# LPD-EPFL/ByzantineMomentum

Hardware: AMD Instinct MI355X
Metric: aggregations/sec (Byzantine-robust GAR over n workers x d dims; achieved HBM GB/s per GAR in roofline/per_gar) (higher is better)
Workload: dtype f32

## Files before the change

### byzantinemomentum_amd/csrc/anticge.hip

```cpp
#include "rank_body.h"
#include "table_sum.h"

namespace bm {

constexpr int kAcgScaleBlock = 256;
constexpr int kAcgMaxBlocks = 256 * 32;
constexpr Caps kAcgCaps = caps_of(kAcgMaxBlocks);
constexpr int kAcgScaleBlocks = 2048;

__global__ __launch_bounds__(64) void anticge_rank_kernel(const double* __restrict__ row_sq, int h, int maxpos,
                                                          int32_t* __restrict__ order, int32_t* __restrict__ order_out,
                                                          double* __restrict__ scal_out) {
  __shared__ double keys[BM_MAX_ROWS];
  __shared__ int32_t ranked[BM_MAX_ROWS];
  const int i = threadIdx.x;
  double key = i < h ? row_sq[i] : 0.0;
  if (!(__builtin_fabs(key) < __builtin_inf())) key = __builtin_inf();
  stable_argsort_body(key, h, keys, ranked);
  __syncthreads();
  order[i] = i < h ? ranked[i] : 0;
  if (order_out != nullptr) order_out[i] = i < h ? ranked[i] : 0;
  if (i == 0) scal_out[1] = keys[ranked[maxpos]];
}

template <int VEC>
__global__ __launch_bounds__(kTableBlock) void anticge_sum_kernel(RowTable rows, const int32_t* __restrict__ order,
                                                                int maxpos, int64_t nvec, float* __restrict__ out,
                                                                int tail, double* __restrict__ partial) {
  __shared__ const float* sel[BM_MAX_ROWS];
  __shared__ double red[kTableBlock / 64];
  const int m = maxpos > 0 ? maxpos : 1;
  if ((int)threadIdx.x < m) sel[threadIdx.x] = rows.p[load_index_coherent(order + threadIdx.x) & (BM_MAX_ROWS - 1)];
  __syncthreads();
  double wide = 0.0;
  table_sum_plain<VEC>(sel, m, nvec, tail, out, AnticgeFold{maxpos > 0}, [&](float x) { wide += (double)x * (double)x; });
  const double r = block_reduce_sum<kTableBlock>(wide, red);
  if (threadIdx.x == 0) partial[blockIdx.x] = r;
}

__global__ __launch_bounds__(64) void anticge_finish_kernel(const double* __restrict__ partial, int nparts,
                                                            double* __restrict__ scal_out) {
  const int lane = threadIdx.x;
  double tot = 0.0;
  for (int b = lane; b < nparts; b += 64) tot += partial[b];
#pragma unroll
  for (int off = 32; off > 0; off >>= 1) tot += __shfl_down(tot, off, 64);
  if (lane == 0) scal_out[0] = tot;
}

__device__ __forceinline__ bool anticge_multiplier(const double* __restrict__ scal, float* mult) {
  const float attnorm = (float)sqrt(scal[0]);
  if (!(attnorm > 0.0f)) return false;
  const float byznorm = (float)sqrt(scal[1]);
  const double norm = (__builtin_fabsf(byznorm) < __builtin_inff()) ? (double)byznorm : __builtin_inf();
  *mult = (float)(-nextafter(norm, 0.0) / (double)attnorm);
  return true;
}

template <int VEC>
__global__ __launch_bounds__(kAcgScaleBlock) void anticge_scale_kernel(float* __restrict__ vec, int64_t nvec,
                                                                  const double* __restrict__ scal) {
  float mult;
  if (!anticge_multiplier(scal, &mult)) return;
  using T = typename VecLoad<VEC>::T;
  const int64_t stride = (int64_t)gridDim.x * kAcgScaleBlock;
  for (int64_t v = (int64_t)blockIdx.x * kAcgScaleBlock + threadIdx.x; v < nvec; v += stride) {
    T x = *reinterpret_cast<const T*>(vec + v * VEC);
    if constexpr (VEC == 1) {
      x = x * mult;
    } else {
#pragma unroll
      for (int c = 0; c < VEC; ++c) x[c] = x[c] * mult;
    }
    *reinterpret_cast<T*>(vec + v * VEC) = x;
  }
}

constexpr int64_t kAcgOrderBytes = BM_MAX_ROWS * (int64_t)sizeof(int32_t);

}

extern "C" int64_t bm_anticge_workspace_bytes(int64_t d) {
  using namespace bm;
  if (d < 0) return BM_EINVAL;
  const int64_t pieces = piece_count(d) > 0 ? piece_count(d) : 1;
  return kAcgOrderBytes + pieces * kAcgCaps.sets() * (int64_t)sizeof(double);
}

extern "C" int bm_anticge_sum(const float* const* rows, int h, int64_t d, int f_decl, const double* row_sq,
                              float* sum_out, int32_t* order_out, double* scal_out, void* ws, void* stream) {
  using namespace bm;
  if (rows == nullptr || row_sq == nullptr || scal_out == nullptr || ws == nullptr || h < 1 || h > BM_MAX_ROWS ||
      f_decl < 1 || f_decl > h || d < 0 || (d > 0 && sum_out == nullptr))
    return BM_EINVAL;
  for (int i = 0; i < h && d > 0; ++i)
    if (rows[i] == nullptr) return BM_EINVAL;
  hipStream_t s = static_cast<hipStream_t>(stream);
  const int maxpos = h - f_decl;
  int32_t* order = static_cast<int32_t*>(ws);
  double* partial = reinterpret_cast<double*>(static_cast<char*>(ws) + kAcgOrderBytes);
  hipLaunchKernelGGL(anticge_rank_kernel, dim3(1), dim3(64), 0, s, row_sq, h, maxpos, order, order_out, scal_out);
  BM_LAUNCH_CHECK();
  RowTable tab{};
  for (int i = 0; i < h; ++i) tab.p[i] = rows[i];
  const int vec = Alignment().of(rows, h).of(sum_out).vec();
  int nparts = 0;
  const int rc = for_pieces(d, [&](int64_t lo, int64_t dp) {
    return for_body_and_tail<4>(Tail::kRidesNarrowed, vec, dp, kTableBlock, kAcgCaps, [&](auto width, const Span& sp) {
      hipLaunchKernelGGL(anticge_sum_kernel<decltype(width)::value>, dim3(sp.grid), dim3(kTableBlock), 0, s,
                         tab.advanced(lo), order, maxpos, sp.count, sum_out + lo, sp.tail, partial + sp.part);
      BM_LAUNCH_CHECK();
      return 0;
    }, &nparts);
  });
  if (rc != 0) return rc;
  hipLaunchKernelGGL(anticge_finish_kernel, dim3(1), dim3(64), 0, s, partial, nparts, scal_out);
  BM_LAUNCH_CHECK();
  return 0;
}

extern "C" int bm_anticge_scale(float* vec, int64_t d, const double* scal, void* stream) {
  using namespace bm;
  if (scal == nullptr || d < 0 || (d > 0 && vec == nullptr)) return BM_EINVAL;
  if (d == 0) return 0;
  hipStream_t s = static_cast<hipStream_t>(stream);
  return for_body_and_tail<4>(Tail::kOwnLaunch, Alignment().of(vec).vec(), d, kAcgScaleBlock, caps_of(kAcgScaleBlocks),
                              [&](auto width, const Span& sp) {
    hipLaunchKernelGGL(anticge_scale_kernel<decltype(width)::value>, dim3(sp.grid), dim3(kAcgScaleBlock), 0, s,
                       vec + sp.first, sp.count, scal);
    BM_LAUNCH_CHECK();
    return 0;
  });
}
```

### byzantinemomentum_amd/csrc/api.cpp

```cpp
#include <stdlib.h>
#include <string.h>
#include <math.h>
#include <algorithm>
#include <vector>
#include "bm_common.h"

namespace bm {
static int env_int(const char* name, int dflt) {
  const char* v = getenv(name);
  if (v == nullptr || *v == '\0') return dflt;
  return atoi(v);
}
static double env_double(const char* name, double dflt) {
  const char* v = getenv(name);
  if (v == nullptr || *v == '\0') return dflt;
  return atof(v);
}
Tuning& tuning_mutable() {
  static Tuning t = {env_int("BM_COL_BURST", 8),  env_int("BM_MEAN_BURST", 8),
                           env_int("BM_STEP_BURST", 8), env_int("BM_STEP_STREAM", 0), env_int("BM_PAIR_MODE", 0),
                           env_int("BM_PAIR_PLANES", 0), env_int("BM_PAIR_DITHER", 0), env_double("BM_PAIR_TAU", 2e-3),
                           env_int("BM_STUDY_BURST", 8), env_int("BM_STEP_STAGGER_US", 0),
                           env_int("BM_GRAM_STEADY", 1), env_int("BM_BULYAN_SHORT", 1),
                           env_int("BM_PAIR_LOAD_NT", 1), env_int("BM_RANK_ALGO", 0), env_int("BM_COL_WIDE", 1), env_int("BM_BRUTE_BUDGET", 0),
                           env_int("BM_WSUM_PIECE", 0), env_int("BM_SPECTRAL_LANES", 0),
                           env_int("BM_PERTURB_GRID", 0)};
  return t;
}
const Tuning& tuning() { return tuning_mutable(); }
}

extern "C" int bm_abi_version(void) { return 23; }

extern "C" int bm_tuning_set(const char* name, int value) {
  using namespace bm;
  if (name == nullptr) return BM_EINVAL;
  Tuning& t = tuning_mutable();
  const struct { const char* key; int* slot; } knobs[] = {
      {"BM_COL_BURST", &t.col_burst}, {"BM_MEAN_BURST", &t.mean_burst}, {"BM_STEP_BURST", &t.step_burst},
      {"BM_STEP_STREAM", &t.step_stream}, {"BM_PAIR_MODE", &t.pair_mode}, {"BM_PAIR_PLANES", &t.pair_planes},
      {"BM_PAIR_DITHER", &t.pair_dither}, {"BM_STUDY_BURST", &t.study_burst},
      {"BM_STEP_STAGGER_US", &t.step_stagger_us}, {"BM_GRAM_STEADY", &t.gram_steady},
      {"BM_BULYAN_SHORT", &t.bulyan_short}, {"BM_PAIR_LOAD_NT", &t.pair_load_nt},
      {"BM_RANK_ALGO", &t.rank_algo}, {"BM_COL_WIDE", &t.col_wide}, {"BM_BRUTE_BUDGET", &t.brute_budget},
      {"BM_WSUM_PIECE", &t.wsum_piece}, {"BM_SPECTRAL_LANES", &t.spectral_lanes},
      {"BM_PERTURB_GRID", &t.perturb_grid}};
  for (const auto& k : knobs)
    if (strcmp(name, k.key) == 0) {
      *k.slot = value;
      return 0;
    }
  return BM_EINVAL;
}

extern "C" const char* bm_error_string(int code) {
  if (code == 0) return "success";
  if (code == BM_EINVAL) return "invalid argument for libbm_gar";
  if (code == BM_ENOCOMM) return "RCCL is not available in this process (librccl.so.1 could not be bound)";
  if (code == BM_ECOMM) return "an RCCL call failed";
  if (code < 0) return hipGetErrorString(static_cast<hipError_t>(-code));
  return "unknown libbm_gar status";
}

namespace {
struct BruteGraph {
  int n;
  uint64_t adj[BM_MAX_ROWS];

  void build(const double* dist, double t) {
    for (int i = 0; i < n; ++i) adj[i] = 0;
    for (int i = 0; i < n; ++i)
      for (int j = i + 1; j < n; ++j) {
        const double v = dist[i * n + j];
        if (isfinite(v) && v <= t) {
          adj[i] |= (uint64_t)1 << j;
          adj[j] |= (uint64_t)1 << i;
        }
      }
  }

  bool has_clique(uint64_t cand, int need) const {
    const int count = __builtin_popcountll(cand);
    if (count < need) return false;
    if (need <= 1) return true;
    int worst = -1, worst_missing = 0;
    for (uint64_t rest = cand; rest != 0; rest &= rest - 1) {
      const int u = __builtin_ctzll(rest);
      const int missing = __builtin_popcountll(cand & ~adj[u] & ~((uint64_t)1 << u));
      if (missing > worst_missing) {
        worst = u;
        worst_missing = missing;
      }
    }
    if (worst < 0) return true;
    const int budget = count - need;
    if (budget == 0) return false;
    const uint64_t bit = (uint64_t)1 << worst;
    if (worst_missing <= budget && has_clique(cand & (adj[worst] | bit), need)) return true;
    return has_clique(cand & ~bit, need);
  }
};
}

extern "C" int bm_brute_select(const double* dist_nxn, int n, int f, int32_t* sel_out) {
  if (dist_nxn == nullptr || sel_out == nullptr || n < 1 || n > BM_MAX_ROWS || f < 0 || n - f < 1)
    return BM_EINVAL;
  const int k = n - f;
  const uint64_t everyone = n == 64 ? ~(uint64_t)0 : (((uint64_t)1 << n) - 1);
  std::vector<double> values;
  values.reserve((size_t)n * (n - 1) / 2 + 1);
  values.push_back(0.0);
  for (int i = 0; i < n; ++i)
    for (int j = i + 1; j < n; ++j) {
      const double v = dist_nxn[i * n + j];
      if (isfinite(v) && v > 0.0) values.push_back(v);
    }
  std::sort(values.begin(), values.end());
  values.erase(std::unique(values.begin(), values.end()), values.end());
  BruteGraph g;
  g.n = n;
  g.build(dist_nxn, values.back());
  if (!g.has_clique(everyone, k)) return BM_EINVAL;
  size_t lo = 0, hi = values.size() - 1;
  while (lo < hi) {
    const size_t mid = (lo + hi) / 2;
    g.build(dist_nxn, values[mid]);
    if (g.has_clique(everyone, k))
      hi = mid;
    else
      lo = mid + 1;
  }
  g.build(dist_nxn, values[lo]);
  uint64_t cand = everyone;
  int chosen = 0;
  for (int c = 0; c < n && chosen < k; ++c) {
    const uint64_t bit = (uint64_t)1 << c;
    if ((cand & bit) == 0) continue;
    const uint64_t above = c == 63 ? 0 : ~(((uint64_t)1 << (c + 1)) - 1);
    const uint64_t next = cand & g.adj[c] & above;
    if (g.has_clique(next, k - chosen - 1)) {
      sel_out[chosen++] = c;
      cand = next;
    }
  }
  return chosen == k ? 0 : BM_EINVAL;
}
```

### byzantinemomentum_amd/csrc/bm_common.h

```cpp
#pragma once
#include <hip/hip_runtime.h>
#include <stdint.h>
#include <utility>
#include "../../include/bm_gar.h"
#include "launch_plan.h"

namespace bm {

struct RowTable {
  const float* p[BM_MAX_ROWS];
  RowTable advanced(int64_t by) const {
    RowTable t = *this;
    advance(t.p, by);
    return t;
  }
};

static inline int hip_code(hipError_t e) { return e == hipSuccess ? 0 : -(int)e; }

#define BM_LAUNCH_CHECK()                      \
  do {                                         \
    hipError_t e__ = hipGetLastError();        \
    if (e__ != hipSuccess) return hip_code(e__); \
  } while (0)

template <int N>
struct MergeExchange {
  static constexpr int kMax = (N < 2) ? 1 : (N * 10);
  struct Table {
    short a[kMax];
    short b[kMax];
    int count;
  };
  static constexpr Table make() {
    Table t{};
    t.count = 0;
    if (N < 2) return t;
    int tt = 0;
    while ((1 << tt) < N) ++tt;
    for (int p = 1 << (tt - 1); p > 0; p /= 2) {
      int q = 1 << (tt - 1), r = 0, d = p;
      while (true) {
        for (int i = 0; i < N - d; ++i)
          if ((i & p) == r) {
            t.a[t.count] = (short)i;
            t.b[t.count] = (short)(i + d);
            ++t.count;
          }
        if (q == p) break;
        d = q - p;
        q /= 2;
        r = p;
      }
    }
    return t;
  }
  static constexpr Table table = make();
};

__device__ __forceinline__ void cmp_exchange(float& a, float& b) {
  float lo, hi;
  asm("v_min_f32 %0, %1, %2" : "=v"(lo) : "v"(a), "v"(b));
  asm("v_max_f32 %0, %1, %2" : "=v"(hi) : "v"(a), "v"(b));
  a = lo;
  b = hi;
}

template <int N, size_t... I>
__device__ __forceinline__ void sort_network_impl(float (&x)[N], std::index_sequence<I...>) {
  (cmp_exchange(x[MergeExchange<N>::table.a[I]], x[MergeExchange<N>::table.b[I]]), ...);
}

template <int N>
__device__ __forceinline__ void sort_network(float (&x)[N]) {
  if constexpr (N >= 2)
    sort_network_impl<N>(x, std::make_index_sequence<MergeExchange<N>::table.count>{});
}

__device__ __forceinline__ float div_small_int(float x, float m, float rm) {
  const float q = x * rm;
  const float r = __builtin_fmaf(-q, m, x);
  const float q1 = __builtin_fmaf(r, rm, q);
  return (q1 == q1) ? q1 : q;
}

template <int VEC>
struct VecLoad;
template <>
struct VecLoad<4> {
  using T = float __attribute__((ext_vector_type(4)));
};
template <>
struct VecLoad<2> {
  using T = float __attribute__((ext_vector_type(2)));
};
template <>
struct VecLoad<1> {
  using T = float;
};

template <int VEC>
__device__ __forceinline__ void load_stream(const float* p, float (&dst)[VEC]) {
  using T = typename VecLoad<VEC>::T;
  const T v = __builtin_nontemporal_load(reinterpret_cast<const T*>(p));
  if constexpr (VEC == 1) {
    dst[0] = v;
  } else {
#pragma unroll
    for (int c = 0; c < VEC; ++c) dst[c] = v[c];
  }
}

template <int VEC>
__device__ __forceinline__ void load_stream_off(const float* base, uint32_t byte_off, float (&dst)[VEC]) {
  load_stream<VEC>(reinterpret_cast<const float*>(reinterpret_cast<const char*>(base) + byte_off), dst);
}

template <int VEC>
__device__ __forceinline__ void store_stream_off(float* base, uint32_t byte_off, const float (&src)[VEC]);

template <int VEC>
__device__ __forceinline__ void store_stream(float* p, const float (&src)[VEC]) {
  using T = typename VecLoad<VEC>::T;
  T v;
  if constexpr (VEC == 1) {
    v = src[0];
  } else {
#pragma unroll
    for (int c = 0; c < VEC; ++c) v[c] = src[c];
  }
  __builtin_nontemporal_store(v, reinterpret_cast<T*>(p));
}

template <int VEC>
__device__ __forceinline__ void store_stream_off(float* base, uint32_t byte_off, const float (&src)[VEC]) {
  store_stream<VEC>(reinterpret_cast<float*>(reinterpret_cast<char*>(base) + byte_off), src);
}

template <int VEC>
__device__ __forceinline__ void store_result(float* p, const float (&src)[VEC]) {
  using T = typename VecLoad<VEC>::T;
  T v;
  if constexpr (VEC == 1) {
    v = src[0];
  } else {
#pragma unroll
    for (int c = 0; c < VEC; ++c) v[c] = src[c];
  }
  *reinterpret_cast<T*>(p) = v;
}
template <int VEC>
__device__ __forceinline__ void store_result_off(float* base, uint32_t byte_off, const float (&src)[VEC]) {
  store_result<VEC>(reinterpret_cast<float*>(reinterpret_cast<char*>(base) + byte_off), src);
}
template <int VEC>
__device__ __forceinline__ void store_result_policy(float* p, const float (&src)[VEC], int nt) {
  if (nt)
    store_stream<VEC>(p, src);
  else
    store_result<VEC>(p, src);
}

constexpr int kColMaxBlocks = 256 * 64;

static inline int lds_opt_in(const void* kernel, size_t dynamic_bytes, size_t static_bytes) {
  if (dynamic_bytes + static_bytes <= 48u * 1024u) return 0;
  return hip_code(hipFuncSetAttribute(kernel, hipFuncAttributeMaxDynamicSharedMemorySize, (int)dynamic_bytes));
}

static inline int compute_units() {
  static int cached[16] = {0};
  int dev = 0;
  if (hipGetDevice(&dev) != hipSuccess || dev < 0 || dev >= 16) dev = 0;
  if (cached[dev] == 0) {
    int cus = 0;
    if (hipDeviceGetAttribute(&cus, hipDeviceAttributeMultiprocessorCount, dev) != hipSuccess || cus <= 0) cus = 256;
    cached[dev] = cus;
  }
  return cached[dev];
}

__device__ __forceinline__ bool arrive_last(int* counter, int total, int* lds_flag) {
  asm volatile("s_waitcnt vmcnt(0)" ::: "memory");
  __syncthreads();
  if (threadIdx.x == 0) {
    __builtin_amdgcn_fence(__ATOMIC_RELEASE, "agent");
    asm volatile("s_waitcnt vmcnt(0)" ::: "memory");
    const int ticket = atomicAdd(counter, 1);
    const int last = (ticket == total - 1) ? 1 : 0;
    if (last) __builtin_amdgcn_fence(__ATOMIC_ACQUIRE, "agent");
    *lds_flag = last;
  }
  __syncthreads();
  return *lds_flag != 0;
}

__device__ __forceinline__ int32_t load_index_coherent(const int32_t* p) {
  return __hip_atomic_load(p, __ATOMIC_RELAXED, __HIP_MEMORY_SCOPE_AGENT);
}

template <int BLOCK>
__device__ __forceinline__ double block_reduce_sum(double v, double* lds ) {
#pragma unroll
  for (int off = 32; off > 0; off >>= 1) v += __shfl_down(v, off, 64);
  const int wave = threadIdx.x >> 6, lane = threadIdx.x & 63;
  if (lane == 0) lds[wave] = v;
  __syncthreads();
  double r = 0.0;
  if (threadIdx.x == 0) {
#pragma unroll
    for (int w = 0; w < BLOCK / 64; ++w) r += lds[w];
  }
  __syncthreads();
  return r;
}

__device__ __forceinline__ float byzantine_coordinate(float avg, float q, float fk, float scale, int attack_kind) {
  const float dir = ((attack_kind & 15) == BM_ATTACK_LITTLE) ? __builtin_sqrtf(q / (fk - 1.0f)) : -avg;
  const float att = dir * scale;
  return (attack_kind & BM_ATTACK_DIRECTION) ? att : avg + att;
}

}

namespace bm {
struct Tuning {
  int col_burst;
  int mean_burst;
  int step_burst;
  int step_stream;
  int pair_mode;
  int pair_planes;
  int pair_dither;
  double pair_tau;
  int study_burst;
  int step_stagger_us;
  int gram_steady;
  int bulyan_short;
  int pair_load_nt;
  int rank_algo;
  int col_wide;
  int brute_budget;
  int wsum_piece;
  int spectral_lanes;
  int perturb_grid;
};
const Tuning& tuning();
Tuning& tuning_mutable();
}
```

### byzantinemomentum_amd/csrc/table_sum.h

```cpp
#pragma once
#include "bm_common.h"

namespace bm {

constexpr int kTableBlock = 256;
struct MeanFold {
  static constexpr bool kFromFirstRow = false;
  float fm;
  __device__ __forceinline__ float start(float) const { return 0.0f; }
  __device__ __forceinline__ float fold(int, float x, float acc) const { return acc + x; }
  __device__ __forceinline__ float finish(float acc) const { return acc / fm; }
};
struct AnticgeFold {
  static constexpr bool kFromFirstRow = true;
  bool twice;
  __device__ __forceinline__ float start(float x) const { return twice ? x + x : x; }
  __device__ __forceinline__ float fold(int, float x, float acc) const { return acc + x; }
  __device__ __forceinline__ float finish(float acc) const { return acc; }
};
struct WeightedFold {
  static constexpr bool kFromFirstRow = false;
  const float* wt;
  float init;
  __device__ __forceinline__ float start(float) const { return init; }
  __device__ __forceinline__ float fold(int k, float x, float acc) const { return __builtin_fmaf(wt[k], x, acc); }
  __device__ __forceinline__ float finish(float acc) const { return acc; }
};
struct NoObserver { __device__ __forceinline__ void operator()(float) const {} };

template <int VEC, class Fold>
__device__ __forceinline__ void table_columns(const float* const* sel, int m, int64_t v, const Fold& f, float (&acc)[VEC]) {
  int k = 0;
  for (int c = 0; c < VEC; ++c) acc[c] = 0.0f;
  if constexpr (Fold::kFromFirstRow) load_stream<VEC>(sel[k++] + v * VEC, acc);
  for (int c = 0; c < VEC; ++c) acc[c] = f.start(acc[c]);
#pragma unroll 8
  for (; k < m; ++k) {
    float t[VEC];
    load_stream<VEC>(sel[k] + v * VEC, t);
    for (int c = 0; c < VEC; ++c) acc[c] = f.fold(k, t[c], acc[c]);
  }
  for (int c = 0; c < VEC; ++c) acc[c] = f.finish(acc[c]);
}

template <int VEC, class Fold, class Observe>
__device__ __forceinline__ void table_sum_tail(const float* const* sel, int m, int64_t nvec, int tail,
                                               float* __restrict__ out, const Fold& f, Observe&& observe) {
  if (VEC > 1 && blockIdx.x == gridDim.x - 1 && (int)threadIdx.x < tail) {
    const int64_t j = nvec * VEC + threadIdx.x;
    int k = 0;
    float acc = 0.0f;
    if constexpr (Fold::kFromFirstRow) acc = sel[k++][j];
    acc = f.start(acc);
    for (; k < m; ++k) acc = f.fold(k, sel[k][j], acc);
    out[j] = acc = f.finish(acc);
    observe(acc);
  }
}

template <int VEC, class Fold, class Observe = NoObserver>
__device__ __forceinline__ void table_sum_plain(const float* const* sel, int m, int64_t nvec, int tail,
                                                float* __restrict__ out, const Fold& f, Observe&& observe = Observe{}) {
  const int64_t nblk = (nvec + kTableBlock - 1) / kTableBlock;
  for (int64_t b = blockIdx.x; b < nblk; b += gridDim.x) {
    const int64_t v = b * kTableBlock + threadIdx.x;
    if (v >= nvec) continue;
    float acc[VEC];
    table_columns<VEC>(sel, m, v, f, acc);
    store_stream<VEC>(out + v * VEC, acc);
    for (int c = 0; c < VEC; ++c) observe(acc[c]);
  }
  table_sum_tail<VEC>(sel, m, nvec, tail, out, f, observe);
}

template <int THREADS, int SLOTS, class Fold>
__device__ __forceinline__ void table_sum_burst(const float* const* sel, int m, int64_t nvec, int tail,
                                                float* __restrict__ out, const Fold& f) {
  using V = typename VecLoad<4>::T;
  __shared__ V stage[SLOTS * THREADS];
  const uint32_t tid = threadIdx.x, nv = (uint32_t)nvec, span = gridDim.x * THREADS;
  const uint32_t iters = (nv + span - 1) / span, first = blockIdx.x * THREADS + tid;
  for (uint32_t p0 = 0; p0 < iters; p0 += SLOTS) {
    const uint32_t p1 = (p0 + SLOTS < iters) ? p0 + SLOTS : iters;
    for (uint32_t it = p0; it < p1; ++it) {
      const uint32_t v = it * span + first;
      if (v < nv) {
        float acc[4];
        table_columns<4>(sel, m, (int64_t)v, f, acc);
        stage[(it - p0) * THREADS + tid] = V{acc[0], acc[1], acc[2], acc[3]};
      }
    }
    __syncthreads();
    for (uint32_t it = p0; it < p1; ++it) {
      const uint32_t v = it * span + first;
      if (v < nv) __builtin_nontemporal_store(stage[(it - p0) * THREADS + tid], reinterpret_cast<V*>(out) + v);
    }
  }
  table_sum_tail<4>(sel, m, nvec, tail, out, f, NoObserver{});
}

}
```

### byzantinemomentum_amd/csrc/weighted_sum.hip

```cpp
#include "table_sum.h"

namespace bm {

constexpr int kWsumMaxBlocks = 256 * 32;

struct RowGroups {
  uint8_t first[BM_MAX_ROWS];
};

__device__ __forceinline__ int weighted_sum_prologue(const RowTable& rows, const RowGroups& groups,
                                                     const double* __restrict__ weights, int n, const float** sel,
                                                     float* wt, double* wd, int* count) {
  const int tid = threadIdx.x;
  if (tid < BM_MAX_ROWS) wd[tid] = tid < n ? weights[tid] : 0.0;
  __syncthreads();
  if (tid < 64) {
    const bool lead = tid < n && groups.first[tid] == tid;
    float g = 0.0f;
    if (lead) {
      double s = 0.0;
      for (int j = tid; j < n; ++j) s += (groups.first[j] == tid) ? wd[j] : 0.0;
      g = (float)s;
    }
    const bool active = lead && g != 0.0f;
    const bool bad = (tid < n && wd[tid] != wd[tid]) || (lead && g != g);
    const unsigned long long mask = __builtin_amdgcn_ballot_w64(active);
    const unsigned long long poison = __builtin_amdgcn_ballot_w64(bad);
    if (active) {
      const int pos = __builtin_popcountll(mask & ((1ull << tid) - 1ull));
      sel[pos] = rows.p[tid];
      wt[pos] = g;
    }
    if (tid == 0) *count = poison != 0ull ? -1 : __builtin_popcountll(mask);
  }
  __syncthreads();
  return *count;
}

template <int VEC>
__global__ __launch_bounds__(kTableBlock) void weighted_sum_kernel(RowTable rows, RowGroups groups,
                                                                   const double* __restrict__ weights, int n,
                                                                   int64_t nvec, float* __restrict__ out, int tail) {
  __shared__ const float* sel[BM_MAX_ROWS];
  __shared__ float wt[BM_MAX_ROWS];
  __shared__ double wd[BM_MAX_ROWS];
  __shared__ int count;
  const int found = weighted_sum_prologue(rows, groups, weights, n, sel, wt, wd, &count);
  const int m = found < 0 ? 0 : found;
  const float init = found < 0 ? __builtin_nanf("") : 0.0f;
  table_sum_plain<VEC>(sel, m, nvec, tail, out, WeightedFold{wt, init});
}

}

extern "C" int bm_weighted_sum(const float* const* rows, int n, const double* weights_dev, int64_t d, float* out,
                               void* stream) {
  using namespace bm;
  if (rows == nullptr || weights_dev == nullptr || (out == nullptr && d > 0) || n < 1 || n > BM_MAX_ROWS || d < 0)
    return BM_EINVAL;
  if (d == 0) return 0;
  hipStream_t s = static_cast<hipStream_t>(stream);
  RowTable tab{};
  RowGroups grp{};
  for (int i = 0; i < n; ++i) {
    tab.p[i] = rows[i];
    int first = i;
    for (int j = 0; j < i; ++j)
      if (rows[j] == rows[i]) {
        first = j;
        break;
      }
    grp.first[i] = (uint8_t)first;
  }
  const int64_t piece = tuning().wsum_piece > 0 ? (int64_t)tuning().wsum_piece : kMaxColsPerLaunch;
  return for_pieces(d, [&](int64_t lo, int64_t dp) {
    const RowTable t = tab.advanced(lo);
    float* const o = out + lo;
    const int vec = Alignment().of(t.p, n).of(o).vec();
    return for_body_and_tail<4>(Tail::kRidesNarrowed, vec, dp, kTableBlock, caps_of(kWsumMaxBlocks), [&](auto width, const Span& sp) {
      hipLaunchKernelGGL(weighted_sum_kernel<decltype(width)::value>, dim3(sp.grid), dim3(kTableBlock), 0, s, t, grp,
                         weights_dev, n, sp.count, o, sp.tail);
      BM_LAUNCH_CHECK();
      return 0;
    });
  }, piece);
}
```

Measured before the change: 5300.

## Route anticge and weighted-sum through persistent burst kernels with staged stores

Adds persistent one-block-per-CU burst kernels (1024 threads, 9 staging slots in shared memory) for the anticge sum and for weighted_sum. Each block computes column sums into an LDS stage and then writes them out with nontemporal stores. table_sum_burst is extended with an observer so anticge can still accumulate its squared norm. The new path is gated by env-tunable burst thresholds on per-CU work. The intent is to raise memory-level parallelism and cut the overhead of many small blocks, at the cost of large LDS use and low occupancy per CU.

```diff
diff --git a/byzantinemomentum_amd/csrc/anticge.hip b/byzantinemomentum_amd/csrc/anticge.hip
--- a/byzantinemomentum_amd/csrc/anticge.hip
+++ b/byzantinemomentum_amd/csrc/anticge.hip
@@ -36,6 +36,42 @@
   table_sum_plain<VEC>(sel, m, nvec, tail, out, AnticgeFold{maxpos > 0}, [&](float x) { wide += (double)x * (double)x; });
   const double r = block_reduce_sum<kTableBlock>(wide, red);
   if (threadIdx.x == 0) partial[blockIdx.x] = r;
+}
+
+__global__ __launch_bounds__(kTableBurstThreads) void anticge_sum_burst_kernel(RowTable rows, const int32_t* __restrict__ order,
+                                                                              int maxpos, int64_t nvec,
+                                                                              float* __restrict__ out, int tail,
+                                                                              double* __restrict__ partial) {
+  __shared__ const float* sel[BM_MAX_ROWS];
+  __shared__ double red[kTableBurstThreads / 64];
+  const int m = maxpos > 0 ? maxpos : 1;
+  if ((int)threadIdx.x < m) sel[threadIdx.x] = rows.p[load_index_coherent(order + threadIdx.x) & (BM_MAX_ROWS - 1)];
+  __syncthreads();
+  double wide = 0.0;
+  table_sum_burst<kTableBurstThreads, kTableBurstSlots>(sel, m, nvec, tail, out, AnticgeFold{maxpos > 0},
+                                                        [&](float x) { wide += (double)x * (double)x; });
+  const double r = block_reduce_sum<kTableBurstThreads>(wide, red);
+  if (threadIdx.x == 0) partial[blockIdx.x] = r;
+}
+
+template <int VEC>
+static int launch_anticge_sum(const RowTable& t, const int32_t* order, int maxpos, Span& sp, float* o, double* partial,
+                              hipStream_t s) {
+  if constexpr (VEC == 4) {
+    const int burst = tuning().acg_burst, cus = compute_units();
+    if (burst > 0 && sp.count < ((int64_t)1 << 30) && cus <= kAcgCaps.body &&
+        (burst == 1 || sp.count / ((int64_t)cus * kTableBurstThreads) >= burst)) {
+      sp.grid = cus;
+      hipLaunchKernelGGL(anticge_sum_burst_kernel, dim3(cus), dim3(kTableBurstThreads), 0, s, t, order, maxpos, sp.count,
+                         o, sp.tail, partial + sp.part);
+      BM_LAUNCH_CHECK();
+      return 0;
+    }
+  }
+  hipLaunchKernelGGL(anticge_sum_kernel<VEC>, dim3(sp.grid), dim3(kTableBlock), 0, s, t, order, maxpos, sp.count, o,
+                     sp.tail, partial + sp.part);
+  BM_LAUNCH_CHECK();
+  return 0;
 }
 
 __global__ __launch_bounds__(64) void anticge_finish_kernel(const double* __restrict__ partial, int nparts,
@@ -106,11 +142,8 @@
   const int vec = Alignment().of(rows, h).of(sum_out).vec();
   int nparts = 0;
   const int rc = for_pieces(d, [&](int64_t lo, int64_t dp) {
-    return for_body_and_tail<4>(Tail::kRidesNarrowed, vec, dp, kTableBlock, kAcgCaps, [&](auto width, const Span& sp) {
-      hipLaunchKernelGGL(anticge_sum_kernel<decltype(width)::value>, dim3(sp.grid), dim3(kTableBlock), 0, s,
-                         tab.advanced(lo), order, maxpos, sp.count, sum_out + lo, sp.tail, partial + sp.part);
-      BM_LAUNCH_CHECK();
-      return 0;
+    return for_body_and_tail<4>(Tail::kRidesNarrowed, vec, dp, kTableBlock, kAcgCaps, [&](auto width, Span& sp) {
+      return launch_anticge_sum<decltype(width)::value>(tab.advanced(lo), order, maxpos, sp, sum_out + lo, partial, s);
     }, &nparts);
   });
   if (rc != 0) return rc;
diff --git a/byzantinemomentum_amd/csrc/api.cpp b/byzantinemomentum_amd/csrc/api.cpp
--- a/byzantinemomentum_amd/csrc/api.cpp
+++ b/byzantinemomentum_amd/csrc/api.cpp
@@ -24,7 +24,7 @@
                            env_int("BM_GRAM_STEADY", 1), env_int("BM_BULYAN_SHORT", 1),
                            env_int("BM_PAIR_LOAD_NT", 1), env_int("BM_RANK_ALGO", 0), env_int("BM_COL_WIDE", 1), env_int("BM_BRUTE_BUDGET", 0),
                            env_int("BM_WSUM_PIECE", 0), env_int("BM_SPECTRAL_LANES", 0),
-                           env_int("BM_PERTURB_GRID", 0)};
+                           env_int("BM_PERTURB_GRID", 0), env_int("BM_WSUM_BURST", 3), env_int("BM_ACG_BURST", 4)};
   return t;
 }
 const Tuning& tuning() { return tuning_mutable(); }
@@ -44,7 +44,7 @@
       {"BM_BULYAN_SHORT", &t.bulyan_short}, {"BM_PAIR_LOAD_NT", &t.pair_load_nt},
       {"BM_RANK_ALGO", &t.rank_algo}, {"BM_COL_WIDE", &t.col_wide}, {"BM_BRUTE_BUDGET", &t.brute_budget},
       {"BM_WSUM_PIECE", &t.wsum_piece}, {"BM_SPECTRAL_LANES", &t.spectral_lanes},
-      {"BM_PERTURB_GRID", &t.perturb_grid}};
+      {"BM_PERTURB_GRID", &t.perturb_grid}, {"BM_WSUM_BURST", &t.wsum_burst}, {"BM_ACG_BURST", &t.acg_burst}};
   for (const auto& k : knobs)
     if (strcmp(name, k.key) == 0) {
       *k.slot = value;
diff --git a/byzantinemomentum_amd/csrc/bm_common.h b/byzantinemomentum_amd/csrc/bm_common.h
--- a/byzantinemomentum_amd/csrc/bm_common.h
+++ b/byzantinemomentum_amd/csrc/bm_common.h
@@ -244,6 +244,8 @@
   int wsum_piece;
   int spectral_lanes;
   int perturb_grid;
+  int wsum_burst;
+  int acg_burst;
 };
 const Tuning& tuning();
 Tuning& tuning_mutable();
diff --git a/byzantinemomentum_amd/csrc/table_sum.h b/byzantinemomentum_amd/csrc/table_sum.h
--- a/byzantinemomentum_amd/csrc/table_sum.h
+++ b/byzantinemomentum_amd/csrc/table_sum.h
@@ -4,6 +4,8 @@
 namespace bm {
 
 constexpr int kTableBlock = 256;
+constexpr int kTableBurstThreads = 1024;
+constexpr int kTableBurstSlots = 9;
 struct MeanFold {
   static constexpr bool kFromFirstRow = false;
   float fm;
@@ -73,9 +75,9 @@
   table_sum_tail<VEC>(sel, m, nvec, tail, out, f, observe);
 }
 
-template <int THREADS, int SLOTS, class Fold>
+template <int THREADS, int SLOTS, class Fold, class Observe = NoObserver>
 __device__ __forceinline__ void table_sum_burst(const float* const* sel, int m, int64_t nvec, int tail,
-                                                float* __restrict__ out, const Fold& f) {
+                                                float* __restrict__ out, const Fold& f, Observe&& observe = Observe{}) {
   using V = typename VecLoad<4>::T;
   __shared__ V stage[SLOTS * THREADS];
   const uint32_t tid = threadIdx.x, nv = (uint32_t)nvec, span = gridDim.x * THREADS;
@@ -88,6 +90,7 @@
         float acc[4];
         table_columns<4>(sel, m, (int64_t)v, f, acc);
         stage[(it - p0) * THREADS + tid] = V{acc[0], acc[1], acc[2], acc[3]};
+        for (int c = 0; c < 4; ++c) observe(acc[c]);
       }
     }
     __syncthreads();
@@ -96,7 +99,7 @@
       if (v < nv) __builtin_nontemporal_store(stage[(it - p0) * THREADS + tid], reinterpret_cast<V*>(out) + v);
     }
   }
-  table_sum_tail<4>(sel, m, nvec, tail, out, f, NoObserver{});
+  table_sum_tail<4>(sel, m, nvec, tail, out, f, observe);
 }
 
 }
diff --git a/byzantinemomentum_amd/csrc/weighted_sum.hip b/byzantinemomentum_amd/csrc/weighted_sum.hip
--- a/byzantinemomentum_amd/csrc/weighted_sum.hip
+++ b/byzantinemomentum_amd/csrc/weighted_sum.hip
@@ -51,6 +51,41 @@
   table_sum_plain<VEC>(sel, m, nvec, tail, out, WeightedFold{wt, init});
 }
 
+__global__ __launch_bounds__(kTableBurstThreads) void weighted_sum_burst_kernel(RowTable rows, RowGroups groups,
+                                                                               const double* __restrict__ weights, int n,
+                                                                               int64_t nvec, float* __restrict__ out,
+                                                                               int tail) {
+  __shared__ const float* sel[BM_MAX_ROWS];
+  __shared__ float wt[BM_MAX_ROWS];
+  __shared__ double wd[BM_MAX_ROWS];
+  __shared__ int count;
+  const int found = weighted_sum_prologue(rows, groups, weights, n, sel, wt, wd, &count);
+  const int m = found < 0 ? 0 : found;
+  const float init = found < 0 ? __builtin_nanf("") : 0.0f;
+  table_sum_burst<kTableBurstThreads, kTableBurstSlots>(sel, m, nvec, tail, out, WeightedFold{wt, init});
+}
+
+constexpr int kWsumBurstMinRows = 8;
+
+template <int VEC>
+static int launch_weighted_sum(const RowTable& t, const RowGroups& grp, const double* weights_dev, int n, int distinct,
+                               const Span& sp, float* o, hipStream_t s) {
+  if constexpr (VEC == 4) {
+    const int burst = tuning().wsum_burst, cus = compute_units();
+    if (burst > 0 && sp.count < ((int64_t)1 << 30) &&
+        (burst == 1 || (distinct >= kWsumBurstMinRows && sp.count / ((int64_t)cus * kTableBurstThreads) >= burst))) {
+      hipLaunchKernelGGL(weighted_sum_burst_kernel, dim3(cus), dim3(kTableBurstThreads), 0, s, t, grp, weights_dev, n,
+                         sp.count, o, sp.tail);
+      BM_LAUNCH_CHECK();
+      return 0;
+    }
+  }
+  hipLaunchKernelGGL(weighted_sum_kernel<VEC>, dim3(sp.grid), dim3(kTableBlock), 0, s, t, grp, weights_dev, n, sp.count,
+                     o, sp.tail);
+  BM_LAUNCH_CHECK();
+  return 0;
+}
+
 }
 
 extern "C" int bm_weighted_sum(const float* const* rows, int n, const double* weights_dev, int64_t d, float* out,
@@ -62,6 +97,7 @@
   hipStream_t s = static_cast<hipStream_t>(stream);
   RowTable tab{};
   RowGroups grp{};
+  int distinct = 0;
   for (int i = 0; i < n; ++i) {
     tab.p[i] = rows[i];
     int first = i;
@@ -71,6 +107,7 @@
         break;
       }
     grp.first[i] = (uint8_t)first;
+    distinct += first == i;
   }
   const int64_t piece = tuning().wsum_piece > 0 ? (int64_t)tuning().wsum_piece : kMaxColsPerLaunch;
   return for_pieces(d, [&](int64_t lo, int64_t dp) {
@@ -78,10 +115,7 @@
     float* const o = out + lo;
     const int vec = Alignment().of(t.p, n).of(o).vec();
     return for_body_and_tail<4>(Tail::kRidesNarrowed, vec, dp, kTableBlock, caps_of(kWsumMaxBlocks), [&](auto width, const Span& sp) {
-      hipLaunchKernelGGL(weighted_sum_kernel<decltype(width)::value>, dim3(sp.grid), dim3(kTableBlock), 0, s, t, grp,
-                         weights_dev, n, sp.count, o, sp.tail);
-      BM_LAUNCH_CHECK();
-      return 0;
+      return launch_weighted_sum<decltype(width)::value>(t, grp, weights_dev, n, distinct, sp, o, s);
     });
   }, piece);
 }
```

Result: no change. 5282 (median of 4 runs) (-0.3%).
